# vwxyzjn/cleanrl

Measured on NVIDIA H100. Metric: env steps/sec (SPS) PPO Breakout num_envs=1024, higher is better.
Workload: dtype bf16

## Files before the change

### cleanrl_b200/csrc/tc_common.cuh

```cuda
#pragma once
#include <cuda_bf16.h>
#include <cstdint>
#include "tc_wgmma.cuh"

namespace b200rl { namespace tc {

__device__ __forceinline__ uint32_t smem_u32(const void* p) {
    return static_cast<uint32_t>(__cvta_generic_to_shared(p));
}

__device__ __forceinline__ void mbar_init(uint64_t* bar, uint32_t count) {
    asm volatile("mbarrier.init.shared::cta.b64 [%0], %1;" ::"r"(smem_u32(bar)), "r"(count) : "memory");
}
__device__ __forceinline__ void fence_barrier_init() {
    asm volatile("fence.mbarrier_init.release.cluster;" ::: "memory");
}
__device__ __forceinline__ bool mbar_try_wait(uint64_t* bar, uint32_t parity) {
    uint32_t ok;
    asm volatile(
        "{\n\t.reg .pred p;\n\t"
        "mbarrier.try_wait.parity.shared::cta.b64 p, [%1], %2;\n\t"
        "selp.u32 %0, 1, 0, p;\n\t}\n"
        : "=r"(ok)
        : "r"(smem_u32(bar)), "r"(parity)
        : "memory");
    return ok != 0;
}
#ifndef B200RL_WAIT_MODE
#define B200RL_WAIT_MODE 0
#endif
__device__ __forceinline__ bool mbar_try_wait_hint(uint64_t* bar, uint32_t parity, uint32_t ns) {
    uint32_t ok;
    asm volatile(
        "{\n\t.reg .pred p;\n\t"
        "mbarrier.try_wait.parity.shared::cta.b64 p, [%1], %2, %3;\n\t"
        "selp.u32 %0, 1, 0, p;\n\t}\n"
        : "=r"(ok)
        : "r"(smem_u32(bar)), "r"(parity), "r"(ns)
        : "memory");
    return ok != 0;
}
__device__ __forceinline__ void mbar_wait(uint64_t* bar, uint32_t parity) {
    if (mbar_try_wait(bar, parity)) return;
    const long long t0 = clock64();
#if B200RL_WAIT_MODE == 1
    while (!mbar_try_wait_hint(bar, parity, 1000000u)) {
#elif B200RL_WAIT_MODE == 2
    while (!mbar_try_wait(bar, parity)) {
        __nanosleep(40);
#else
    while (!mbar_try_wait(bar, parity)) {
#endif
        if (clock64() - t0 > (1ll << 33)) __trap();
    }
}

__device__ __forceinline__ void mbar_wait2(uint64_t* bar_a, uint32_t parity_a, uint64_t* bar_b, uint32_t parity_b) {
    const bool a = mbar_try_wait(bar_a, parity_a), b = mbar_try_wait(bar_b, parity_b);
    if (a && b) return;
    if (!a) mbar_wait(bar_a, parity_a);
    if (!b) mbar_wait(bar_b, parity_b);
}

__device__ __forceinline__ void st_global_32b(void* p, const int4& a, const int4& b) {
    reinterpret_cast<int4*>(p)[0] = a;
    reinterpret_cast<int4*>(p)[1] = b;
}

__device__ __forceinline__ void fence_proxy_async_smem() {
    asm volatile("fence.proxy.async.shared::cta;" ::: "memory");
}

constexpr uint64_t kDescSwizzle128 = 1ull << 62;
constexpr uint64_t kDescSwizzle64 = 2ull << 62;

__device__ __forceinline__ uint64_t desc_kmajor(uint32_t smem_addr) {
    return (uint64_t)((smem_addr & 0x3FFFFu) >> 4) | (1ull << 16) | (64ull << 32) | kDescSwizzle128;
}
__device__ __forceinline__ uint64_t desc_mnmajor(uint32_t smem_addr, uint32_t lbo_bytes) {
    return (uint64_t)((smem_addr & 0x3FFFFu) >> 4) | ((uint64_t)((lbo_bytes >> 4) & 0x3FFF) << 16) | (64ull << 32) |
           kDescSwizzle128;
}

template <int R>
__device__ __forceinline__ void stage_acc(float* st, int ld, int wg_tid, const float (&d)[R]) {
    const int row = ((wg_tid >> 5) << 4) + ((wg_tid & 31) >> 2), col = (wg_tid & 3) * 2;
#pragma unroll
    for (int j = 0; j < R / 4; ++j) {
        *reinterpret_cast<float2*>(st + row * ld + 8 * j + col) = make_float2(d[4 * j], d[4 * j + 1]);
        *reinterpret_cast<float2*>(st + (row + 8) * ld + 8 * j + col) = make_float2(d[4 * j + 2], d[4 * j + 3]);
    }
}
__device__ __forceinline__ void named_bar(int id, int n) { asm volatile("bar.sync %0, %1;" ::"r"(id), "r"(n) : "memory"); }

__device__ __forceinline__ uint32_t img_off(int r, int c) { return (uint32_t)(r * 128 + ((c ^ (r & 7)) << 4)); }

__device__ __forceinline__ uint32_t pack_bf16x2_relu(float lo, float hi) {
    uint32_t d;
    asm("cvt.rn.relu.bf16x2.f32 %0, %1, %2;" : "=r"(d) : "f"(hi), "f"(lo));
    return d;
}
__device__ __forceinline__ uint32_t pack_bf16x2(float lo, float hi) {
    __nv_bfloat162 v = __floats2bfloat162_rn(lo, hi);
    return *reinterpret_cast<uint32_t*>(&v);
}

}}

namespace b200rl { namespace tc {
__device__ __forceinline__ void cp_async16(uint32_t smem_addr, const void* gptr, uint32_t src_bytes) {
    asm volatile("cp.async.cg.shared.global [%0], [%1], 16, %2;" ::"r"(smem_addr), "l"(gptr), "r"(src_bytes) : "memory");
}
__device__ __forceinline__ void cp_async_commit() { asm volatile("cp.async.commit_group;" ::: "memory"); }
template <int N>
__device__ __forceinline__ void cp_async_wait() { asm volatile("cp.async.wait_group %0;" ::"n"(N) : "memory"); }
__device__ __forceinline__ void mbar_arrive(uint64_t* bar) {
    asm volatile("mbarrier.arrive.shared::cta.b64 _, [%0];" ::"r"(smem_u32(bar)) : "memory");
}
}}

namespace b200rl { namespace tc {
__device__ __forceinline__ void tma_load_2d(uint32_t smem_dst, const void* tmap, int x, int y, uint64_t* bar) {
    asm volatile("cp.async.bulk.tensor.2d.shared::cluster.global.mbarrier::complete_tx::bytes [%0], [%1, {%2, %3}], [%4];"
                 ::"r"(smem_dst), "l"(reinterpret_cast<uint64_t>(tmap)), "r"(x), "r"(y), "r"(smem_u32(bar))
                 : "memory");
}
__device__ __forceinline__ void tma_load_3d(uint32_t smem_dst, const void* tmap, int x, int y, int z, uint64_t* bar) {
    asm volatile("cp.async.bulk.tensor.3d.shared::cluster.global.mbarrier::complete_tx::bytes [%0], [%1, {%2, %3, %4}], [%5];"
                 ::"r"(smem_dst), "l"(reinterpret_cast<uint64_t>(tmap)), "r"(x), "r"(y), "r"(z), "r"(smem_u32(bar))
                 : "memory");
}
__device__ __forceinline__ void mbar_arrive_expect_tx(uint64_t* bar, uint32_t bytes) {
    asm volatile("mbarrier.arrive.expect_tx.shared::cta.b64 _, [%0], %1;" ::"r"(smem_u32(bar)), "r"(bytes) : "memory");
}
__device__ __forceinline__ void tma_prefetch_desc(const void* tmap) {
    asm volatile("prefetch.tensormap [%0];" ::"l"(reinterpret_cast<uint64_t>(tmap)) : "memory");
}
}}
```

### cleanrl_b200/csrc/tc_conv1_u8.cuh

```cuda
#pragma once
#include "tc_base.cuh"
#include <cuda_fp16.h>
#include "tc_conv_win.cuh"

namespace b200rl {
using namespace tc;

__device__ __forceinline__ uint64_t desc_kmajor_sw64(uint32_t smem_addr) {
    return (uint64_t)((smem_addr & 0x3FFFFu) >> 4) | (1ull << 16) | (32ull << 32) | kDescSwizzle64;
}
__device__ __forceinline__ uint64_t desc_mnmajor_sw64(uint32_t smem_addr, uint32_t lbo) {
    return (uint64_t)((smem_addr & 0x3FFFFu) >> 4) | ((uint64_t)((lbo >> 4) & 0x3FFF) << 16) | (32ull << 32) | kDescSwizzle64;
}
__device__ __forceinline__ uint32_t img64_off(int r, int c) { return (uint32_t)(r * 64 + ((c ^ ((r >> 1) & 3)) << 4)); }
__global__ void __launch_bounds__(256) tc_frames_to_s2d_u8(const uint8_t* __restrict__ obs, const int64_t* __restrict__ rows, int64_t n,
                                                           uint8_t* __restrict__ out_rm, uint8_t* __restrict__ out_cm) {
    __shared__ __align__(16) uint8_t plane[7056];
    const int64_t i = blockIdx.x >> 2;
    const int c = blockIdx.x & 3;
    const int64_t img = rows ? rows[i] : i;
    const int4* src = reinterpret_cast<const int4*>(obs + img * 28224 + c * 7056);
    for (int t = threadIdx.x; t < 441; t += 256) reinterpret_cast<int4*>(plane)[t] = __ldg(src + t);
    __syncthreads();
    for (int pos = threadIdx.x; pos < 441; pos += 256) {
// ... 77 lines not shown
    if (tid == 0) {
        for (int s = 0; s < STAGES; ++s) { mbar_init(&full_bar[s], 1); mbar_init(&empty_bar[s], 8); }
        fence_barrier_init();
        tma_prefetch_desc(&tmA);
    }
    for (int idx = tid; idx < NTAPS * BN * 4; idx += blockDim.x) {
        const int c16 = idx & 3;
        const int t = (idx >> 2) & 3;
        const int r = idx >> 4;
        *reinterpret_cast<int4*>(sW + t * B_CHUNK + img64_off(r, c16)) = ldg16(p.limbs + r * 256 + t * 64 + c16 * 16);
    }
    if (tid < 32) { s_sc[tid] = p.sc[32 + tid]; s_bias[tid] = p.bias[tid]; }
    fence_proxy_async_smem();
    __syncthreads();
    const int tile_begin = (int)(((int64_t)total_tiles * blockIdx.x) / gridDim.x);
    const int tile_end = (int)(((int64_t)total_tiles * (blockIdx.x + 1)) / gridDim.x);

    if (warp == 0) {
        if (tid == 0) {
            uint32_t q = 0;
            int z_next = 0;
            if (tile_begin < tile_end) {
                const int img = tile_begin >> 1;
                z_next = p.rows ? (int)__ldg(p.rows + img) : img;
            }
            for (int tile = tile_begin; tile < tile_end; ++tile, ++q) {
                const uint32_t s = q % STAGES;
                const int z = z_next;
                if (tile + 1 < tile_end) {
                    const int img = (tile + 1) >> 1;
                    z_next = p.rows ? (int)__ldg(p.rows + img) : img;
                }
                if (q >= (uint32_t)STAGES) mbar_wait(&empty_bar[s], ((q / STAGES) - 1) & 1);
                mbar_arrive_expect_tx(&full_bar[s], (uint32_t)STAGE_BYTES);
                tma_load_3d(smem_u32(sRing + (size_t)s * STAGE_BYTES), &tmA, 0, (tile & 1) * 128, z, &full_bar[s]);
            }
        }
    } else if (warp >= 4) {
        const int wg = (warp - 4) >> 2, wt = tid & 127, lane = tid & 31, qd = lane & 3;
        const uint32_t w_base = smem_u32(sW);
        constexpr int off[4] = {0, 1, 21, 22};
        int acc[2][32];
#pragma unroll
        for (int e = 0; e < 2; ++e)
#pragma unroll
            for (int c = 0; c < 32; ++c) acc[e][c] = 0;
        for (int tile = tile_begin; tile < tile_end; ++tile) {
            const uint32_t q = (uint32_t)(tile - tile_begin), s = q % STAGES;
            mbar_wait(&full_bar[s], (q / STAGES) & 1);
            wgmma_fence();
            const uint32_t win = smem_u32(sRing + (size_t)s * STAGE_BYTES) + (uint32_t)(wg * 64 * 128);
#pragma unroll
            for (int e = 0; e < 2; ++e) {
#pragma unroll
                for (int t = 0; t < NTAPS; ++t) {
                    const int po = e + off[t];
                    const uint64_t a = desc_kmajor(win + (uint32_t)((po >> 1) * 128 + (po & 1) * 64));
                    const uint64_t b = desc_kmajor_sw64(w_base + (uint32_t)(t * B_CHUNK));
#pragma unroll
                    for (int kk = 0; kk < 2; ++kk) wgmma_u8s8_n64(acc[e], a + 2 * kk, b + 2 * kk, (t | kk) != 0 ? 1u : 0u);
                }
            }
            wgmma_commit();
            wgmma_wait<0>();
            wgmma_fence_operands(acc[0]);
            wgmma_fence_operands(acc[1]);
            if (lane == 0) mbar_arrive(&empty_bar[s]);
            const int i = tile >> 1;
#pragma unroll
            for (int e = 0; e < 2; ++e) {
#pragma unroll
                for (int hr = 0; hr < 2; ++hr) {
                    const int lrow = wg * 64 + ((wt >> 5) << 4) + (lane >> 2) + 8 * hr;
                    const int rem = 2 * (((tile & 1) << 7) + lrow) + e;
                    const int Y = (rem * 3121) >> 16, X = rem - Y * 21;
                    const bool valid = rem < 441 && Y < 20 && X < 20;
                    const int64_t cell = ((int64_t)i * 10 + (Y >> 1)) * 10 + (X >> 1);
                    const int cls = (Y & 1) * 2 + (X & 1);
                    uint32_t bits = 0u, pk[4];
#pragma unroll
                    for (int j = 0; j < 4; ++j) {
                        const int co = 8 * j + 2 * qd;
                        const float f0 = fmaf((float)(acc[e][4 * j + 2 * hr] * 128 + acc[e][4 * (j + 4) + 2 * hr]), s_sc[co], s_bias[co]);
                        const float f1 = fmaf((float)(acc[e][4 * j + 2 * hr + 1] * 128 + acc[e][4 * (j + 4) + 2 * hr + 1]), s_sc[co + 1],
                                              s_bias[co + 1]);
                        bits |= (f0 > 0.f ? 1u : 0u) << co;
                        bits |= (f1 > 0.f ? 1u : 0u) << (co + 1);
                        pk[j] = pack_bf16x2_relu(f0, f1);
                    }
                    bits |= __shfl_xor_sync(0xffffffffu, bits, 1);
                    bits |= __shfl_xor_sync(0xffffffffu, bits, 2);
                    if (valid) {
                        if (qd == 0) p.mask_out[cell * 4 + cls] = bits;
                        uint32_t* dst = reinterpret_cast<uint32_t*>(reinterpret_cast<uint8_t*>(p.out) + (cell * 4 + cls) * 64);
#pragma unroll
                        for (int j = 0; j < 4; ++j) dst[4 * j + qd] = pk[j];
                    }
                }
            }
        }
    }
}

struct Conv21BwdU8Params {
    const int64_t* rows;
    int n;
    int64_t rows_per_cta;
    const bf16* w2dg;
    const uint32_t* m1;
    float* ws;
    float* wsb;
};
constexpr int kC1WXStages = 6, kC21WinStages = 2;
constexpr int kC1WBlock = 64 * 128, kC1WYBytes = 128 * 64, kC1WYPadRows = 24, kC1WYPad = kC1WYPadRows * 64;
constexpr int kC1WShift = 21;
constexpr int kC21WinRows = 140, kC21WinBytes = 18 * 1024;
constexpr int kC21W2Bytes = 4 * 128 * 128;
constexpr int kC21ImgBytes = kC1WYPad + 4 * kC1WYBytes;
constexpr float kDact1Scale = 4096.0f;

__device__ __forceinline__ uint32_t prmt(uint32_t a, uint32_t b, uint32_t sel) {
    uint32_t d;
    asm("prmt.b32 %0, %1, %2, %3;" : "=r"(d) : "r"(a), "r"(b), "r"(sel));
    return d;
}
constexpr float kU8Bias = 1024.0f;


__device__ __forceinline__ uint32_t pair_f16_biased(const uint32_t (&w)[5], int j, bool up, uint32_t sel) {
    const uint32_t lo = up ? w[j + 1] : w[j];
    const uint32_t hi = up ? w[j + 2] : w[j + 1];
    return prmt(prmt(lo, hi, sel), 0x64646464u, 0x5140u);
}
__device__ __forceinline__ uint4 lds128(uint32_t addr) {
    uint4 v;
    asm volatile("ld.shared.v4.u32 {%0, %1, %2, %3}, [%4];" : "=r"(v.x), "=r"(v.y), "=r"(v.z), "=r"(v.w) : "r"(addr) : "memory");
    return v;
}
__device__ __forceinline__ uint32_t pack_f16x2_sat(float lo, float hi) {
    uint32_t d;
    asm("cvt.rn.satfinite.f16x2.f32 %0, %1, %2;" : "=r"(d) : "f"(hi), "f"(lo));
    return d;
}

__device__ __forceinline__ void sts32(uint32_t addr, uint32_t v) { asm volatile("st.shared.u32 [%0], %1;" ::"r"(addr), "r"(v) : "memory"); }
__device__ __forceinline__ void tma_store_3d(const void* tmap, uint32_t smem_src, int x, int y, int z) {
    asm volatile("cp.async.bulk.tensor.3d.global.shared::cta.bulk_group [%0, {%1, %2, %3}], [%4];"
                 ::"l"(reinterpret_cast<uint64_t>(tmap)), "r"(x), "r"(y), "r"(z), "r"(smem_src) : "memory");
}
__device__ __forceinline__ void bulk_commit() { asm volatile("cp.async.bulk.commit_group;" ::: "memory"); }
template <int N> __device__ __forceinline__ void bulk_wait_read() { asm volatile("cp.async.bulk.wait_group.read %0;" ::"n"(N) : "memory"); }
template <int N> __device__ __forceinline__ void bulk_wait() { asm volatile("cp.async.bulk.wait_group %0;" ::"n"(N) : "memory"); }

template <int R> __device__ __forceinline__ void setmaxnreg_dec() { asm volatile("setmaxnreg.dec.sync.aligned.u32 %0;" ::"n"(R)); }
template <int R> __device__ __forceinline__ void setmaxnreg_inc() { asm volatile("setmaxnreg.inc.sync.aligned.u32 %0;" ::"n"(R)); }
constexpr int kC1WRegsProducer = 40, kC21RegsDgrad = 128, kC1WRegsMma = 168;
static_assert(128 * kC1WRegsProducer + 128 * kC21RegsDgrad + 256 * kC1WRegsMma <= 65536, "register budgets exceed the SM");

constexpr int kC1WThreads = 512;
__global__ void __launch_bounds__(kC1WThreads, 1) tc_conv21_bwd_u8(const __grid_constant__ CUtensorMap tmX, const __grid_constant__ CUtensorMap tmWin,
                                                                 const __grid_constant__ CUtensorMap tmY, const Conv21BwdU8Params p) {
    constexpr int XS = kC1WXStages, WS = kC21WinStages;
    extern __shared__ uint8_t smem_raw[];
    __shared__ uint64_t xfull[XS], xempty[XS], wfull[WS], wempty[WS], yfull[2], yempty[2];
    __shared__ float sRed[32 * 32], sBias[32];
    uint8_t* smem = reinterpret_cast<uint8_t*>((reinterpret_cast<uintptr_t>(smem_raw) + 1023) & ~uintptr_t(1023));
    uint8_t* sW2 = smem;
    uint8_t* sWin = sW2 + kC21W2Bytes;
    uint8_t* sX = sWin + (size_t)WS * kC21WinBytes;
    uint8_t* sImg = sX + (size_t)XS * kC1WBlock;
    const int tid = threadIdx.x, warp = tid >> 5, lane = tid & 31;
    if (tid == 0) {
        for (int s = 0; s < XS; ++s) { mbar_init(&xfull[s], 1); mbar_init(&xempty[s], 12); }
        for (int s = 0; s < WS; ++s) { mbar_init(&wfull[s], 1); mbar_init(&wempty[s], 4); }
        for (int s = 0; s < 2; ++s) { mbar_init(&yfull[s], 1); mbar_init(&yempty[s], 8); }
        fence_barrier_init();
        tma_prefetch_desc(&tmX);
        tma_prefetch_desc(&tmWin);
        tma_prefetch_desc(&tmY);
    }
    for (int idx = tid; idx < 4 * 128 * 8; idx += blockDim.x) {
        const int c16 = idx & 7, r = (idx >> 3) & 127, t = idx >> 10;
        *reinterpret_cast<int4*>(sW2 + t * (128 * 128) + img_off(r, c16)) = ldg16(p.w2dg + r * 256 + t * 64 + c16 * 8);
    }
    for (int idx = tid; idx < 2 * kC21ImgBytes / 16; idx += blockDim.x) reinterpret_cast<int4*>(sImg)[idx] = make_int4(0, 0, 0, 0);
    fence_proxy_async_smem();
    __syncthreads();
    const int64_t M = (int64_t)p.n * 512;
    const int64_t m_begin = (int64_t)blockIdx.x * p.rows_per_cta;
    int64_t m_end = m_begin + p.rows_per_cta;
    if (m_end > M) m_end = M;
    const int nsteps = m_end > m_begin ? (int)((m_end - m_begin) >> 7) : 0;
    const int nimg = nsteps >> 2;
    const int64_t g0 = m_begin >> 7;
    const int img0 = (int)(m_begin >> 9);

    if (warp < 4) {
        setmaxnreg_dec<kC1WRegsProducer>();
        if (warp == 0 && lane == 0 && nsteps > 0) {
            auto image_of = [&](int64_t g) -> int {
                int64_t img = g >> 2;
                if (img >= p.n) img = p.n - 1;
                return p.rows ? (int)__ldg(p.rows + img) : (int)img;
            };
            int z = image_of(g0), z_next = image_of(g0 + 4);
            for (int k = 0; k <= nsteps; ++k) {
                const int64_t g = g0 + k;
                if (k > 0 && (g & 3) == 0) { z = z_next; z_next = image_of(g + 4); }
                const int xs = k % XS;
                if (k >= XS) mbar_wait(&xempty[xs], ((k / XS) - 1) & 1);
                mbar_arrive_expect_tx(&xfull[xs], (uint32_t)kC1WBlock);
                tma_load_3d(smem_u32(sX + (size_t)xs * kC1WBlock), &tmX, (int)(g & 3) * 128, 0, z, &xfull[xs]);
            }
        } else if (warp == 1 && lane == 0) {
            for (int j = 0; j < nimg; ++j) {
                const int s = j % WS;
                if (j >= WS) mbar_wait(&wempty[s], ((j / WS) - 1) & 1);
                mbar_arrive_expect_tx(&wfull[s], (uint32_t)(kC21WinRows * 128));
                tma_load_2d(smem_u32(sWin + (size_t)s * kC21WinBytes), &tmWin, 0, (img0 + j) * 121, &wfull[s]);
            }
        }
    } else if (warp < 8) {
        const int wt = tid - 128, lane4 = lane >> 2, qd = lane & 3;
        const uint32_t w_base = smem_u32(sW2);
        const int rq = wt >> 2, c16 = wt & 3;
        float bsum[8];
#pragma unroll
        for (int e = 0; e < 8; ++e) bsum[e] = 0.f;
        for (int j = 0; j < nimg; ++j) {
            const int i = img0 + j, buf = j & 1, s = j % WS;
            const uint32_t img = smem_u32(sImg + (size_t)buf * kC21ImgBytes) + kC1WYPad;
            mbar_wait(&wfull[s], (j / WS) & 1);
            if (j >= 2) mbar_wait(&yempty[buf], ((j >> 1) - 1) & 1);
            if (wt == 0) bulk_wait_read<1>();
            named_bar(1, 128);
#pragma unroll 1
            for (int h2 = 0; h2 < 2; ++h2) {
                float d[64];
                wgmma_fence();
                const uint32_t win = smem_u32(sWin + (size_t)s * kC21WinBytes) + (uint32_t)(h2 * 64 * 128);
                constexpr int shift[4] = {12, 11, 1, 0};
#pragma unroll
                for (int t = 0; t < 4; ++t) {
                    const uint64_t a = desc_kmajor(win + (uint32_t)shift[t] * 128u);
                    const uint64_t b = desc_kmajor(w_base + (uint32_t)(t * 128 * 128));
#pragma unroll
                    for (int kk = 0; kk < 4; ++kk) WgmmaBf16<128, 0, 0>::mma(d, a + 2 * kk, b + 2 * kk, (t | kk) != 0 ? 1u : 0u);
                }
                wgmma_commit();
                int pos[2];
                uint4 mb[2];
#pragma unroll
                for (int hr = 0; hr < 2; ++hr) {
                    const int r = h2 * 64 + ((wt >> 5) << 4) + lane4 + 8 * hr;
                    const int Y = (r * 5958) >> 16, X = r - Y * 11;
                    const bool valid = Y < 10 && X < 10;
                    pos[hr] = valid ? 2 * Y * 21 + 2 * X : -1;
                    mb[hr] = make_uint4(0u, 0u, 0u, 0u);
                    if (valid) {
                        const int4 t = ldg16(p.m1 + ((int64_t)i * 100 + Y * 10 + X) * 4);
                        mb[hr] = make_uint4((uint32_t)t.x, (uint32_t)t.y, (uint32_t)t.z, (uint32_t)t.w);
                    }
                }
                wgmma_wait<0>();
                wgmma_fence_operands(d);
                if (h2 == 1 && lane == 0) mbar_arrive(&wempty[s]);
#pragma unroll
                for (int hr = 0; hr < 2; ++hr) {
                    if (pos[hr] < 0) continue;
                    const uint32_t mw[4] = {mb[hr].x, mb[hr].y, mb[hr].z, mb[hr].w};
#pragma unroll
                    for (int jj = 0; jj < 16; ++jj) {
                        const int g = jj >> 2, c = 8 * (jj & 3) + 2 * qd;
                        float f0 = d[4 * jj + 2 * hr] * kDact1Scale, f1 = d[4 * jj + 2 * hr + 1] * kDact1Scale;
                        if (!((mw[g] >> c) & 1u)) f0 = 0.f;
                        if (!((mw[g] >> (c + 1)) & 1u)) f1 = 0.f;
                        const int q = pos[hr] + (g >> 1) * 21 + (g & 1);
                        sts32(img + img64_off(q, c >> 3) + (uint32_t)((c & 7) * 2), pack_f16x2_sat(f0, f1));
                    }
                }
            }
            fence_proxy_async_smem();
            named_bar(1, 128);
            if (wt == 0) {
                mbar_arrive(&yfull[buf]);
#pragma unroll
                for (int k = 0; k < 4; ++k) tma_store_3d(&tmY, img + (uint32_t)(k * kC1WYBytes), 0, k * 128, i);
                bulk_commit();
            }
#pragma unroll 1
            for (int st = 0; st < 4; ++st) {
#pragma unroll
                for (int ps = 0; ps < 4; ++ps) {
                    const uint4 v = lds128(img + (uint32_t)(st * kC1WYBytes) + img64_off(ps * 32 + rq, c16));
                    const uint32_t w[4] = {v.x, v.y, v.z, v.w};
#pragma unroll
                    for (int e = 0; e < 4; ++e) {
                        const float2 f = __half22float2(*reinterpret_cast<const __half2*>(&w[e]));
                        bsum[2 * e] += f.x;
                        bsum[2 * e + 1] += f.y;
                    }
                }
            }
        }
        if (wt == 0) bulk_wait<0>();
#pragma unroll
        for (int e = 0; e < 8; ++e) sRed[rq * 32 + c16 * 8 + e] = bsum[e];
        named_bar(1, 128);
// ... 107 lines not shown
```

### cleanrl_b200/csrc/tc_conv_win.cuh

```cuda
#pragma once
#include "tc_base.cuh"

namespace b200rl {
using namespace tc;

enum { WOUT_DENSE = 0, WOUT_S2D2 = 1, WOUT_DACT2 = 2, WOUT_DACT1 = 3 };
struct WinParams {
    const bf16* A;
    const int64_t* rows;
    int64_t M;
    int n, G, Wp;
    int tpi_shift;
    int64_t n_images;
    int ntaps;
    int shift[16];
    int WR;
    const bf16* Bw;
    int N;
    int vH, vW;
    int out_mode;
    bf16* out;
    bf16* out2;
    const uint32_t* mask_bits;
    uint32_t* mask_out;
// ... 97 lines not shown
#pragma unroll
            for (int t = 0; t < NTAPS; ++t) {
#pragma unroll
                for (int c = 0; c < CPR; ++c) {
                    const uint64_t a = desc_kmajor(win + (uint32_t)(c * IMG) + (uint32_t)p.shift[t] * 128u);
                    const uint64_t b = desc_kmajor(w_base + (uint32_t)((t * CPR + c) * B_CHUNK));
#pragma unroll
                    for (int kk = 0; kk < 4; ++kk)
                        WgmmaBf16<BN, 0, 0>::mma(d, a + 2 * kk, b + 2 * kk, (t | c | kk) != 0 ? 1u : 0u);
                }
            }
            wgmma_commit();
            const int Y = (int)(((uint32_t)rem * mW) >> 16), X = rem - Y * p.Wp;
            const bool valid = inside && (Y < p.vH) && (X < p.vW);
            int64_t o1 = 0, ob = 0;
            if (p.out_mode == WOUT_S2D2) {
                const int64_t cell = ((int64_t)i * 10 + (Y >> 1)) * 10 + (X >> 1);
                const int cls = (Y & 1) * 2 + (X & 1);
                o1 = cell * 128 + cls * 32; ob = cell * 4 + cls;
            } else {
                ob = ((int64_t)i * 100 + Y * 10 + X) * 4;
            }
            uint32_t mb[NW];
#pragma unroll
            for (int g = 0; g < NW; ++g) mb[g] = 0xFFFFFFFFu;
            if (p.mask_bits != nullptr && valid) {
                if (NW == 4) {
                    const int4 t = ldg16(p.mask_bits + ob);
                    mb[0] = (uint32_t)t.x; mb[1 % NW] = (uint32_t)t.y; mb[2 % NW] = (uint32_t)t.z; mb[3 % NW] = (uint32_t)t.w;
                } else if (NW == 2) {
                    const uint2 t = __ldg(reinterpret_cast<const uint2*>(p.mask_bits + ob));
                    mb[0] = t.x; mb[1 % NW] = t.y;
                } else {
                    mb[0] = __ldg(p.mask_bits + ob);
                }
            }
            wgmma_wait<0>();
            wgmma_fence_operands(d);
            if ((tid & 31) == 0) mbar_arrive(&empty_bar[s]);
            named_bar(1 + wg, 128);
            stage_acc(st, LDA, wt, d);
            named_bar(1 + wg, 128);
#pragma unroll
            for (int g = 0; g < NW; ++g) {
                if ((g & 1) != half) continue;
                if (!valid || g * 32 >= p.N) continue;
                uint32_t v[32];
#pragma unroll
                for (int e = 0; e < 8; ++e) {
                    const float4 f = *reinterpret_cast<const float4*>(st + lr * LDA + g * 32 + 4 * e);
                    v[4 * e] = __float_as_uint(f.x); v[4 * e + 1] = __float_as_uint(f.y);
                    v[4 * e + 2] = __float_as_uint(f.z); v[4 * e + 3] = __float_as_uint(f.w);
                }
                if (p.bias) {
                    const float4* bp = reinterpret_cast<const float4*>(p.bias + g * 32);
#pragma unroll
                    for (int e = 0; e < 8; ++e) {
                        const float4 bv = __ldg(bp + e);
                        v[4 * e] = __float_as_uint(fmaf(__uint_as_float(v[4 * e]), p.scale, bv.x));
                        v[4 * e + 1] = __float_as_uint(fmaf(__uint_as_float(v[4 * e + 1]), p.scale, bv.y));
                        v[4 * e + 2] = __float_as_uint(fmaf(__uint_as_float(v[4 * e + 2]), p.scale, bv.z));
                        v[4 * e + 3] = __float_as_uint(fmaf(__uint_as_float(v[4 * e + 3]), p.scale, bv.w));
                    }
                } else {
#pragma unroll
                    for (int e = 0; e < 32; ++e) v[e] = __float_as_uint(__uint_as_float(v[e]) * p.scale);
                }
                if (p.relu) {
                    uint32_t bits = 0u;
#pragma unroll
                    for (int e = 0; e < 32; ++e) {
                        const float f = __uint_as_float(v[e]);
                        bits |= (f > 0.f ? 1u : 0u) << e;
                    }
                    if (p.mask_out) p.mask_out[ob + g] = bits;
                }
                if (p.mask_bits) {
#pragma unroll
                    for (int e = 0; e < 32; ++e) if (!((mb[g] >> e) & 1u)) v[e] = 0u;
                }
                int4 w[4];
                if (p.relu) {
#pragma unroll
                    for (int e = 0; e < 4; ++e) {
                        w[e].x = (int)pack_bf16x2_relu(__uint_as_float(v[8 * e]), __uint_as_float(v[8 * e + 1]));
                        w[e].y = (int)pack_bf16x2_relu(__uint_as_float(v[8 * e + 2]), __uint_as_float(v[8 * e + 3]));
                        w[e].z = (int)pack_bf16x2_relu(__uint_as_float(v[8 * e + 4]), __uint_as_float(v[8 * e + 5]));
                        w[e].w = (int)pack_bf16x2_relu(__uint_as_float(v[8 * e + 6]), __uint_as_float(v[8 * e + 7]));
                    }
                } else {
#pragma unroll
                for (int e = 0; e < 4; ++e) {
                    w[e].x = (int)pack_bf16x2(__uint_as_float(v[8 * e]), __uint_as_float(v[8 * e + 1]));
                    w[e].y = (int)pack_bf16x2(__uint_as_float(v[8 * e + 2]), __uint_as_float(v[8 * e + 3]));
                    w[e].z = (int)pack_bf16x2(__uint_as_float(v[8 * e + 4]), __uint_as_float(v[8 * e + 5]));
                    w[e].w = (int)pack_bf16x2(__uint_as_float(v[8 * e + 6]), __uint_as_float(v[8 * e + 7]));
                }
                }
                if (p.out_mode == WOUT_DACT1) {
                    int4* brow = reinterpret_cast<int4*>(st + lr * LDA) + 8 * g + 4 * (g & 1);
#pragma unroll
                    for (int e = 0; e < 4; ++e) brow[e] = w[e];
                } else {
                    bf16* dst = p.out + o1 + g * 32;
                    st_global_32b(dst, w[0], w[1]);
                    st_global_32b(dst + 16, w[2], w[3]);
                }
            }
            if (p.out_mode == WOUT_DACT1) {
                if (half == 0)
                    *reinterpret_cast<int64_t*>(st + lr * LDA + BN) = valid ? ((int64_t)i * 441 + 2 * Y * 21 + 2 * X) * 32 : -1;
                named_bar(1 + wg, 128);
#pragma unroll
                for (int m = 0; m < 8; ++m) {
                    const int k = m * 128 + wt, g = (k >> 2) & 3, e = k & 3;
                    const float* srow = st + (k >> 4) * LDA;
                    const int64_t o = *reinterpret_cast<const int64_t*>(srow + BN);
                    if (o < 0) continue;
                    const int4 val = reinterpret_cast<const int4*>(srow)[8 * g + 4 * (g & 1) + e];
                    *reinterpret_cast<int4*>(p.out + o + (g >> 1) * 21 * 32 + (g & 1) * 32 + e * 8) = val;
                }
            }
        }
    }
}

template <int BN, int CPR, int STAGES, int NTAPS>
static int launch_conv_win(const WinParams& p, cudaStream_t s, const char* what) {
    if (p.ntaps != NTAPS) return fail(B200RL_ERR_INVALID_ARGUMENT, "%s: %d taps, kernel instance has %d", what, p.ntaps, NTAPS);
    if (p.out_mode != WOUT_S2D2 && p.out_mode != WOUT_DACT1)
        return fail(B200RL_ERR_INVALID_ARGUMENT, "%s: dense and conv3 data-gradient outputs run on tc_conv_win_t", what);
    if (p.out_mode == WOUT_DACT1 && (BN != 128 || p.N != 128))
        return fail(B200RL_ERR_INVALID_ARGUMENT, "%s: the conv2 data gradient stores 4 groups of 32 channels per cell", what);
    const size_t smem = (size_t)p.ntaps * CPR * BN * 128 + (size_t)STAGES * p.WR * 128 * CPR + conv_win_acc_bytes<BN>() + 1024;
    static SmemAttrCache attr;
    if (int rc = attr.ensure(tc_conv_win<BN, CPR, STAGES, NTAPS>, smem, what)) return rc;
    if ((int64_t)p.G * p.Wp >= 65536 || p.G < 1 || p.N % 32 != 0)
        return fail(B200RL_ERR_INVALID_ARGUMENT, "%s: grid %d x width %d outside the epilogue's multiply-shift range, or N %% 32 != 0", what, p.G, p.Wp);
    if (p.rows && !p.tpi_shift) return fail(B200RL_ERR_INVALID_ARGUMENT, "%s: the image gather needs image-aligned tiling", what);
    if (p.tpi_shift && (128 << p.tpi_shift) < p.G) return fail(B200RL_ERR_INVALID_ARGUMENT, "%s: tiles per image too small", what);
    const int total = p.tpi_shift ? (int)((int64_t)p.n << p.tpi_shift) : (int)ceil_div(p.M, 128);
    int grid = num_sms();
    if (grid > total) grid = total;
    CUtensorMap tmA;
    memset(&tmA, 0, sizeof(tmA));
    int rc;
    if (p.tpi_shift) rc = make_tmap_3d(&tmA, p.A, p.n_images, p.G, (int64_t)CPR * 64, p.WR, what);
    else rc = make_tmap_2d(&tmA, p.A, p.M, (int64_t)CPR * 64, p.WR, what);
    if (rc) return rc;
    tc_conv_win<BN, CPR, STAGES, NTAPS><<<grid, kConvWinThreads, smem, s>>>(tmA, p, total);
    return check_launch(what);
}

constexpr int kConvWinTThreads = 384;
constexpr int kConvWinTLds = 64 + 4;
template <int BP>
__host__ __device__ constexpr size_t conv_win_t_stage_bytes() { return (size_t)2 * BP * kConvWinTLds * sizeof(float); }

template <int R>
__device__ __forceinline__ void stage_acc_transposed(float* st, int wg_tid, const float (&d)[R]) {
    const int co = ((wg_tid >> 5) << 4) + ((wg_tid & 31) >> 2), pos = (wg_tid & 3) * 2;
#pragma unroll
    for (int j = 0; j < R / 4; ++j) {
        float* p0 = st + (8 * j + pos) * kConvWinTLds + co;
        p0[0] = d[4 * j];
        p0[kConvWinTLds] = d[4 * j + 1];
        p0[8] = d[4 * j + 2];
        p0[kConvWinTLds + 8] = d[4 * j + 3];
    }
}

template <int BP, int CPR, int STAGES, int NTAPS>
__global__ void __launch_bounds__(kConvWinTThreads, 1) tc_conv_win_t(const __grid_constant__ CUtensorMap tmA, const WinParams p,
                                                                     int total_tiles) {
    static_assert(BP % 128 == 0, "one thread per position row of a 128-row slice");
    static_assert(STAGES % 2 == 0, "each consumer warpgroup owns every other stage");
    constexpr int RPT = BP / 128;
    constexpr int A_CHUNK = 64 * 128;
    constexpr int LDS = kConvWinTLds;
    extern __shared__ uint8_t smem_raw[];
    __shared__ uint64_t full_bar[STAGES], empty_bar[STAGES];
    uint8_t* smem = reinterpret_cast<uint8_t*>((reinterpret_cast<uintptr_t>(smem_raw) + 1023) & ~uintptr_t(1023));
    const int tid = threadIdx.x, warp = tid >> 5;
    const int nchunks = NTAPS * CPR;
    const int K = nchunks * 64;
    const int IMG = p.WR * 128;
    const int STAGE_BYTES = IMG * CPR;
    uint8_t* sW = smem;
    uint8_t* sRing = smem + (size_t)nchunks * A_CHUNK;
    float* sAcc = reinterpret_cast<float*>(sRing + (size_t)STAGES * STAGE_BYTES);

    if (tid == 0) {
        for (int s = 0; s < STAGES; ++s) { mbar_init(&full_bar[s], 1); mbar_init(&empty_bar[s], 4); }
        fence_barrier_init();
        tma_prefetch_desc(&tmA);
    }
    for (int idx = tid; idx < nchunks * 64 * 8; idx += blockDim.x) {
        const int c16 = idx & 7;
        const int t = idx >> 3;
        const int r = t & 63, j = t >> 6;
        int4 v = make_int4(0, 0, 0, 0);
        if (r < p.N) v = ldg16(p.Bw + (int64_t)r * K + j * 64 + c16 * 8);
        *reinterpret_cast<int4*>(sW + (size_t)j * A_CHUNK + img_off(r, c16)) = v;
    }
    fence_proxy_async_smem();
    __syncthreads();
    const int tile_begin = (int)(((int64_t)total_tiles * blockIdx.x) / gridDim.x);
    const int tile_end = (int)(((int64_t)total_tiles * (blockIdx.x + 1)) / gridDim.x);

    if (warp == 0) {
        if (tid == 0) {
            uint32_t q = 0;
            for (int tile = tile_begin; tile < tile_end; ++tile, ++q) {
                const uint32_t s = q % STAGES;
                if (q >= (uint32_t)STAGES) mbar_wait(&empty_bar[s], ((q / STAGES) - 1) & 1);
                const uint32_t dst = smem_u32(sRing + (size_t)s * STAGE_BYTES);
                mbar_arrive_expect_tx(&full_bar[s], (uint32_t)STAGE_BYTES);
#pragma unroll
                for (int c = 0; c < CPR; ++c) tma_load_2d(dst + c * IMG, &tmA, c * 64, tile * BP, &full_bar[s]);
            }
        }
    } else if (warp >= 4) {
        const int wg = (warp - 4) >> 2, wt = tid & 127;
        float* st = sAcc + wg * BP * LDS;
        const uint32_t w_base = smem_u32(sW);
        const uint32_t mW = (65536u + (uint32_t)p.Wp - 1u) / (uint32_t)p.Wp;
        constexpr int NW = 2;
        float d[BP / 2];
#pragma unroll
        for (int e = 0; e < BP / 2; ++e) d[e] = 0.f;
        for (int tile = tile_begin + wg; tile < tile_end; tile += 2) {
            const uint32_t q = (uint32_t)(tile - tile_begin), s = q % STAGES;
            mbar_wait(&full_bar[s], (q / STAGES) & 1);
            wgmma_fence();
            const uint32_t win = smem_u32(sRing + (size_t)s * STAGE_BYTES);
#pragma unroll
            for (int t = 0; t < NTAPS; ++t) {
#pragma unroll
                for (int c = 0; c < CPR; ++c) {
                    const uint64_t b = desc_kmajor(win + (uint32_t)(c * IMG) + (uint32_t)p.shift[t] * 128u);
                    const uint64_t a = desc_kmajor(w_base + (uint32_t)((t * CPR + c) * A_CHUNK));
#pragma unroll
                    for (int kk = 0; kk < 4; ++kk)
                        WgmmaBf16<BP, 0, 0>::mma(d, a + 2 * kk, b + 2 * kk, (t | c | kk) != 0 ? 1u : 0u);
                }
            }
            wgmma_commit();
            bool valid[RPT];
            int64_t o1[RPT], o2[RPT], ob[RPT];
            uint32_t mb[RPT][NW];
#pragma unroll
            for (int rr = 0; rr < RPT; ++rr) {
                const int64_t r = (int64_t)tile * BP + rr * 128 + wt;
                const int i = (int)(r / p.G);
                const int rem = (int)(r - (int64_t)i * p.G);
                const int Y = (int)(((uint32_t)rem * mW) >> 16), X = rem - Y * p.Wp;
                valid[rr] = r < p.M && (Y < p.vH) && (X < p.vW);
                o2[rr] = 0;
                if (p.out_mode == WOUT_DENSE) {
                    const int64_t orow = ((int64_t)i * p.vH + Y) * p.vW + X;
                    o1[rr] = orow * p.N; ob[rr] = orow * (p.N >> 5);
                } else {
                    o1[rr] = ((int64_t)i * 100 + Y * 10 + X) * 64;
                    o2[rr] = ((int64_t)i * 121 + (Y + 1) * 11 + (X + 1)) * 64;
                    ob[rr] = ((int64_t)i * 81 + Y * 9 + X) * 2;
                }
                mb[rr][0] = mb[rr][1] = 0xFFFFFFFFu;
                if (p.mask_bits != nullptr && valid[rr]) {
                    const uint2 t = __ldg(reinterpret_cast<const uint2*>(p.mask_bits + ob[rr]));
                    mb[rr][0] = t.x; mb[rr][1] = t.y;
                }
            }
            wgmma_wait<0>();
            wgmma_fence_operands(d);
            if ((tid & 31) == 0) mbar_arrive(&empty_bar[s]);
            named_bar(1 + wg, 128);
            stage_acc_transposed(st, wt, d);
            named_bar(1 + wg, 128);
#pragma unroll
            for (int rr = 0; rr < RPT; ++rr) {
                float* srow = st + (rr * 128 + wt) * LDS;
#pragma unroll
                for (int g = 0; g < NW; ++g) {
                    if (!valid[rr] || g * 32 >= p.N) continue;
                    uint32_t v[32];
#pragma unroll
                    for (int e = 0; e < 8; ++e) {
                        const float4 f = *reinterpret_cast<const float4*>(srow + g * 32 + 4 * e);
                        v[4 * e] = __float_as_uint(f.x); v[4 * e + 1] = __float_as_uint(f.y);
                        v[4 * e + 2] = __float_as_uint(f.z); v[4 * e + 3] = __float_as_uint(f.w);
                    }
                    if (p.bias) {
                        const float4* bp = reinterpret_cast<const float4*>(p.bias + g * 32);
#pragma unroll
                        for (int e = 0; e < 8; ++e) {
                            const float4 bv = __ldg(bp + e);
                            v[4 * e] = __float_as_uint(fmaf(__uint_as_float(v[4 * e]), p.scale, bv.x));
                            v[4 * e + 1] = __float_as_uint(fmaf(__uint_as_float(v[4 * e + 1]), p.scale, bv.y));
                            v[4 * e + 2] = __float_as_uint(fmaf(__uint_as_float(v[4 * e + 2]), p.scale, bv.z));
                            v[4 * e + 3] = __float_as_uint(fmaf(__uint_as_float(v[4 * e + 3]), p.scale, bv.w));
                        }
                    } else {
#pragma unroll
                        for (int e = 0; e < 32; ++e) v[e] = __float_as_uint(__uint_as_float(v[e]) * p.scale);
                    }
                    if (p.relu) {
                        uint32_t bits = 0u;
#pragma unroll
                        for (int e = 0; e < 32; ++e) bits |= (__uint_as_float(v[e]) > 0.f ? 1u : 0u) << e;
                        if (p.mask_out) p.mask_out[ob[rr] + g] = bits;
                    }
                    if (p.mask_bits) {
#pragma unroll
                        for (int e = 0; e < 32; ++e) if (!((mb[rr][g] >> e) & 1u)) v[e] = 0u;
                    }
                    int4 w[4];
                    if (p.relu) {
#pragma unroll
                        for (int e = 0; e < 4; ++e) {
                            w[e].x = (int)pack_bf16x2_relu(__uint_as_float(v[8 * e]), __uint_as_float(v[8 * e + 1]));
                            w[e].y = (int)pack_bf16x2_relu(__uint_as_float(v[8 * e + 2]), __uint_as_float(v[8 * e + 3]));
                            w[e].z = (int)pack_bf16x2_relu(__uint_as_float(v[8 * e + 4]), __uint_as_float(v[8 * e + 5]));
                            w[e].w = (int)pack_bf16x2_relu(__uint_as_float(v[8 * e + 6]), __uint_as_float(v[8 * e + 7]));
                        }
                    } else {
#pragma unroll
                        for (int e = 0; e < 4; ++e) {
                            w[e].x = (int)pack_bf16x2(__uint_as_float(v[8 * e]), __uint_as_float(v[8 * e + 1]));
                            w[e].y = (int)pack_bf16x2(__uint_as_float(v[8 * e + 2]), __uint_as_float(v[8 * e + 3]));
                            w[e].z = (int)pack_bf16x2(__uint_as_float(v[8 * e + 4]), __uint_as_float(v[8 * e + 5]));
                            w[e].w = (int)pack_bf16x2(__uint_as_float(v[8 * e + 6]), __uint_as_float(v[8 * e + 7]));
                        }
                    }
                    int4* brow = reinterpret_cast<int4*>(srow) + 4 * g;
#pragma unroll
                    for (int e = 0; e < 4; ++e) brow[e] = w[e];
                }
                *reinterpret_cast<longlong2*>(srow + 64) = make_longlong2(valid[rr] ? o1[rr] : -1, o2[rr]);
            }
            named_bar(1 + wg, 128);
#pragma unroll
            for (int m = 0; m < BP / 16; ++m) {
                const int k = m * 128 + wt, part = k & 7;
                const float* srow = st + (k >> 3) * LDS;
                const longlong2 off = *reinterpret_cast<const longlong2*>(srow + 64);
                if (off.x < 0) continue;
                const int4 val = reinterpret_cast<const int4*>(srow)[part];
                *reinterpret_cast<int4*>(p.out + off.x + part * 8) = val;
                if (p.out_mode == WOUT_DACT2) *reinterpret_cast<int4*>(p.out2 + off.y + part * 8) = val;
            }
        }
    }
}

template <int BP, int CPR, int STAGES, int NTAPS>
static int launch_conv_win_t(WinParams p, cudaStream_t s, const char* what) {
    if (p.ntaps != NTAPS) return fail(B200RL_ERR_INVALID_ARGUMENT, "%s: %d taps, kernel instance has %d", what, p.ntaps, NTAPS);
    if (p.N != 64) return fail(B200RL_ERR_INVALID_ARGUMENT, "%s: N = %d, the kernel computes 64 output channels", what, p.N);
    if ((int64_t)p.G * p.Wp >= 65536 || p.G < 1)
        return fail(B200RL_ERR_INVALID_ARGUMENT, "%s: grid %d x width %d outside the epilogue's multiply-shift range", what, p.G, p.Wp);
    if (p.rows || p.tpi_shift) return fail(B200RL_ERR_INVALID_ARGUMENT, "%s: the channel-major kernel walks a contiguous linear grid", what);
    if (p.out_mode != WOUT_DENSE && p.out_mode != WOUT_DACT2)
        return fail(B200RL_ERR_INVALID_ARGUMENT, "%s: only bf16 dense and conv3 data-gradient outputs in this kernel", what);
    int maxs = 0;
    for (int t = 0; t < NTAPS; ++t) maxs = p.shift[t] > maxs ? p.shift[t] : maxs;
    p.WR = (BP + maxs + 7) & ~7;
    if (p.WR > 256) return fail(B200RL_ERR_INVALID_ARGUMENT, "%s: window of %d rows exceeds a TMA box", what, p.WR);
    const size_t smem = (size_t)NTAPS * CPR * 64 * 128 + (size_t)STAGES * p.WR * 128 * CPR + conv_win_t_stage_bytes<BP>() + 1024;
    static SmemAttrCache attr;
    if (int rc = attr.ensure(tc_conv_win_t<BP, CPR, STAGES, NTAPS>, smem, what)) return rc;
    const int total = (int)ceil_div(p.M, BP);
    int grid = num_sms();
    if (grid > total) grid = total;
    CUtensorMap tmA;
    memset(&tmA, 0, sizeof(tmA));
    if (int rc = make_tmap_2d(&tmA, p.A, p.M, (int64_t)CPR * 64, p.WR, what)) return rc;
    tc_conv_win_t<BP, CPR, STAGES, NTAPS><<<grid, kConvWinTThreads, smem, s>>>(tmA, p, total);
    return check_launch(what);
}

}
```

Before: 1.192 million.

## Split conv window kernel into producer, MMA and dedicated epilogue warpgroups

Restructures the channel-major windowed conv kernel into five warpgroups: a TMA producer, two MMA warpgroups and two epilogue warpgroups. They hand off through staged and freed mbarriers on double-buffered accumulator staging, so the next tile's MMA can overlap the current tile's epilogue. Registers are rebalanced with setmaxnreg, and weights are loaded by TMA instead of a cooperative global-to-shared copy. Bias is cached in shared memory, and BP is restricted to 128 with a 32-bit position index. The cost is more threads and tighter per-thread register budgets, which risks spills, and a more complex barrier protocol.

```diff
diff --git a/cleanrl_b200/csrc/tc_common.cuh b/cleanrl_b200/csrc/tc_common.cuh
--- a/cleanrl_b200/csrc/tc_common.cuh
+++ b/cleanrl_b200/csrc/tc_common.cuh
@@ -93,6 +93,9 @@
 }
 __device__ __forceinline__ void named_bar(int id, int n) { asm volatile("bar.sync %0, %1;" ::"r"(id), "r"(n) : "memory"); }
 
+template <int R> __device__ __forceinline__ void setmaxnreg_dec() { asm volatile("setmaxnreg.dec.sync.aligned.u32 %0;" ::"n"(R)); }
+template <int R> __device__ __forceinline__ void setmaxnreg_inc() { asm volatile("setmaxnreg.inc.sync.aligned.u32 %0;" ::"n"(R)); }
+
 __device__ __forceinline__ uint32_t img_off(int r, int c) { return (uint32_t)(r * 128 + ((c ^ (r & 7)) << 4)); }
 
 __device__ __forceinline__ uint32_t pack_bf16x2_relu(float lo, float hi) {
diff --git a/cleanrl_b200/csrc/tc_conv1_u8.cuh b/cleanrl_b200/csrc/tc_conv1_u8.cuh
--- a/cleanrl_b200/csrc/tc_conv1_u8.cuh
+++ b/cleanrl_b200/csrc/tc_conv1_u8.cuh
@@ -253,8 +253,6 @@
 template <int N> __device__ __forceinline__ void bulk_wait_read() { asm volatile("cp.async.bulk.wait_group.read %0;" ::"n"(N) : "memory"); }
 template <int N> __device__ __forceinline__ void bulk_wait() { asm volatile("cp.async.bulk.wait_group %0;" ::"n"(N) : "memory"); }
 
-template <int R> __device__ __forceinline__ void setmaxnreg_dec() { asm volatile("setmaxnreg.dec.sync.aligned.u32 %0;" ::"n"(R)); }
-template <int R> __device__ __forceinline__ void setmaxnreg_inc() { asm volatile("setmaxnreg.inc.sync.aligned.u32 %0;" ::"n"(R)); }
 constexpr int kC1WRegsProducer = 40, kC21RegsDgrad = 128, kC1WRegsMma = 168;
 static_assert(128 * kC1WRegsProducer + 128 * kC21RegsDgrad + 256 * kC1WRegsMma <= 65536, "register budgets exceed the SM");
 
diff --git a/cleanrl_b200/csrc/tc_conv_win.cuh b/cleanrl_b200/csrc/tc_conv_win.cuh
--- a/cleanrl_b200/csrc/tc_conv_win.cuh
+++ b/cleanrl_b200/csrc/tc_conv_win.cuh
@@ -273,10 +273,15 @@
     return check_launch(what);
 }
 
-constexpr int kConvWinTThreads = 384;
 constexpr int kConvWinTLds = 64 + 4;
 template <int BP>
 __host__ __device__ constexpr size_t conv_win_t_stage_bytes() { return (size_t)2 * BP * kConvWinTLds * sizeof(float); }
+
+constexpr int kConvWinTThreads = 640;
+constexpr int kConvWinTRegsLaunch = (65536 / kConvWinTThreads) & ~7;
+constexpr int kConvWinTRegsProducer = 24, kConvWinTRegsMma = 112, kConvWinTRegsEpi = 112;
+static_assert(128 * kConvWinTRegsProducer + 256 * kConvWinTRegsMma + 256 * kConvWinTRegsEpi <= kConvWinTRegsLaunch * kConvWinTThreads,
+              "register budgets exceed what the CTA launches with");
 
 template <int R>
 __device__ __forceinline__ void stage_acc_transposed(float* st, int wg_tid, const float (&d)[R]) {
@@ -292,19 +297,20 @@
 }
 
 template <int BP, int CPR, int STAGES, int NTAPS>
-__global__ void __launch_bounds__(kConvWinTThreads, 1) tc_conv_win_t(const __grid_constant__ CUtensorMap tmA, const WinParams p,
-                                                                     int total_tiles) {
-    static_assert(BP % 128 == 0, "one thread per position row of a 128-row slice");
-    static_assert(STAGES % 2 == 0, "each consumer warpgroup owns every other stage");
-    constexpr int RPT = BP / 128;
+__global__ void __launch_bounds__(kConvWinTThreads, 1)
+    tc_conv_win_t(const __grid_constant__ CUtensorMap tmA, const __grid_constant__ CUtensorMap tmW, const WinParams p,
+                  int total_tiles) {
+    static_assert(BP == 128, "one epilogue thread per position row");
+    static_assert(STAGES % 2 == 0, "each MMA warpgroup owns every other stage");
     constexpr int A_CHUNK = 64 * 128;
     constexpr int LDS = kConvWinTLds;
+    constexpr int NW = 2;
     extern __shared__ uint8_t smem_raw[];
-    __shared__ uint64_t full_bar[STAGES], empty_bar[STAGES];
+    __shared__ uint64_t full_bar[STAGES], empty_bar[STAGES], staged_bar[2], freed_bar[2], w_bar;
+    __shared__ __align__(16) float s_bias[2][64];
     uint8_t* smem = reinterpret_cast<uint8_t*>((reinterpret_cast<uintptr_t>(smem_raw) + 1023) & ~uintptr_t(1023));
-    const int tid = threadIdx.x, warp = tid >> 5;
+    const int tid = threadIdx.x, warp = tid >> 5, wgi = warp >> 2, wt = tid & 127;
     const int nchunks = NTAPS * CPR;
-    const int K = nchunks * 64;
     const int IMG = p.WR * 128;
     const int STAGE_BYTES = IMG * CPR;
     uint8_t* sW = smem;
@@ -313,24 +319,21 @@
 
     if (tid == 0) {
         for (int s = 0; s < STAGES; ++s) { mbar_init(&full_bar[s], 1); mbar_init(&empty_bar[s], 4); }
+        for (int b = 0; b < 2; ++b) { mbar_init(&staged_bar[b], 128); mbar_init(&freed_bar[b], 128); }
+        mbar_init(&w_bar, 1);
         fence_barrier_init();
         tma_prefetch_desc(&tmA);
+        tma_prefetch_desc(&tmW);
     }
-    for (int idx = tid; idx < nchunks * 64 * 8; idx += blockDim.x) {
-        const int c16 = idx & 7;
-        const int t = idx >> 3;
-        const int r = t & 63, j = t >> 6;
-        int4 v = make_int4(0, 0, 0, 0);
-        if (r < p.N) v = ldg16(p.Bw + (int64_t)r * K + j * 64 + c16 * 8);
-        *reinterpret_cast<int4*>(sW + (size_t)j * A_CHUNK + img_off(r, c16)) = v;
-    }
-    fence_proxy_async_smem();
     __syncthreads();
     const int tile_begin = (int)(((int64_t)total_tiles * blockIdx.x) / gridDim.x);
     const int tile_end = (int)(((int64_t)total_tiles * (blockIdx.x + 1)) / gridDim.x);
 
-    if (warp == 0) {
-        if (tid == 0) {
+    if (wgi == 0) {
+        setmaxnreg_dec<kConvWinTRegsProducer>();
+        if (tid == 0 && tile_begin < tile_end) {
+            mbar_arrive_expect_tx(&w_bar, (uint32_t)(nchunks * A_CHUNK));
+            for (int j = 0; j < nchunks; ++j) tma_load_2d(smem_u32(sW + (size_t)j * A_CHUNK), &tmW, j * 64, 0, &w_bar);
             uint32_t q = 0;
             for (int tile = tile_begin; tile < tile_end; ++tile, ++q) {
                 const uint32_t s = q % STAGES;
@@ -341,16 +344,17 @@
                 for (int c = 0; c < CPR; ++c) tma_load_2d(dst + c * IMG, &tmA, c * 64, tile * BP, &full_bar[s]);
             }
         }
-    } else if (warp >= 4) {
-        const int wg = (warp - 4) >> 2, wt = tid & 127;
+    } else if (wgi <= 2) {
+        setmaxnreg_inc<kConvWinTRegsMma>();
+        const int wg = wgi - 1;
         float* st = sAcc + wg * BP * LDS;
         const uint32_t w_base = smem_u32(sW);
-        const uint32_t mW = (65536u + (uint32_t)p.Wp - 1u) / (uint32_t)p.Wp;
-        constexpr int NW = 2;
         float d[BP / 2];
 #pragma unroll
         for (int e = 0; e < BP / 2; ++e) d[e] = 0.f;
-        for (int tile = tile_begin + wg; tile < tile_end; tile += 2) {
+        if (tile_begin + wg < tile_end) mbar_wait(&w_bar, 0);
+        uint32_t k = 0;
+        for (int tile = tile_begin + wg; tile < tile_end; tile += 2, ++k) {
             const uint32_t q = (uint32_t)(tile - tile_begin), s = q % STAGES;
             mbar_wait(&full_bar[s], (q / STAGES) & 1);
             wgmma_fence();
@@ -367,109 +371,113 @@
                 }
             }
             wgmma_commit();
-            bool valid[RPT];
-            int64_t o1[RPT], o2[RPT], ob[RPT];
-            uint32_t mb[RPT][NW];
-#pragma unroll
-            for (int rr = 0; rr < RPT; ++rr) {
-                const int64_t r = (int64_t)tile * BP + rr * 128 + wt;
-                const int i = (int)(r / p.G);
-                const int rem = (int)(r - (int64_t)i * p.G);
-                const int Y = (int)(((uint32_t)rem * mW) >> 16), X = rem - Y * p.Wp;
-                valid[rr] = r < p.M && (Y < p.vH) && (X < p.vW);
-                o2[rr] = 0;
-                if (p.out_mode == WOUT_DENSE) {
-                    const int64_t orow = ((int64_t)i * p.vH + Y) * p.vW + X;
-                    o1[rr] = orow * p.N; ob[rr] = orow * (p.N >> 5);
-                } else {
-                    o1[rr] = ((int64_t)i * 100 + Y * 10 + X) * 64;
-                    o2[rr] = ((int64_t)i * 121 + (Y + 1) * 11 + (X + 1)) * 64;
-                    ob[rr] = ((int64_t)i * 81 + Y * 9 + X) * 2;
-                }
-                mb[rr][0] = mb[rr][1] = 0xFFFFFFFFu;
-                if (p.mask_bits != nullptr && valid[rr]) {
-                    const uint2 t = __ldg(reinterpret_cast<const uint2*>(p.mask_bits + ob[rr]));
-                    mb[rr][0] = t.x; mb[rr][1] = t.y;
-                }
-            }
             wgmma_wait<0>();
             wgmma_fence_operands(d);
             if ((tid & 31) == 0) mbar_arrive(&empty_bar[s]);
-            named_bar(1 + wg, 128);
+            if (k > 0) mbar_wait(&freed_bar[wg], (k - 1) & 1);
             stage_acc_transposed(st, wt, d);
-            named_bar(1 + wg, 128);
-#pragma unroll
-            for (int rr = 0; rr < RPT; ++rr) {
-                float* srow = st + (rr * 128 + wt) * LDS;
-#pragma unroll
-                for (int g = 0; g < NW; ++g) {
-                    if (!valid[rr] || g * 32 >= p.N) continue;
-                    uint32_t v[32];
+            mbar_arrive(&staged_bar[wg]);
+        }
+    } else {
+        setmaxnreg_inc<kConvWinTRegsEpi>();
+        const int b = wgi - 3;
+        float* st = sAcc + b * BP * LDS;
+        float* srow = st + wt * LDS;
+        const uint32_t mW = (65536u + (uint32_t)p.Wp - 1u) / (uint32_t)p.Wp;
+        float* sb = s_bias[b];
+        if (p.bias && wt < 64) sb[wt] = __ldg(p.bias + wt);
+        named_bar(1 + b, 128);
+        uint32_t k = 0;
+        for (int tile = tile_begin + b; tile < tile_end; tile += 2, ++k) {
+            const uint32_t r = (uint32_t)tile * BP + (uint32_t)wt;
+            const int i = (int)(r / (uint32_t)p.G);
+            const int rem = (int)(r - (uint32_t)i * (uint32_t)p.G);
+            const int Y = (int)(((uint32_t)rem * mW) >> 16), X = rem - Y * p.Wp;
+            const bool valid = (int64_t)r < p.M && (Y < p.vH) && (X < p.vW);
+            int64_t o1, o2 = 0, ob;
+            if (p.out_mode == WOUT_DENSE) {
+                const int64_t orow = ((int64_t)i * p.vH + Y) * p.vW + X;
+                o1 = orow * p.N; ob = orow * (p.N >> 5);
+            } else {
+                o1 = ((int64_t)i * 100 + Y * 10 + X) * 64;
+                o2 = ((int64_t)i * 121 + (Y + 1) * 11 + (X + 1)) * 64;
+                ob = ((int64_t)i * 81 + Y * 9 + X) * 2;
+            }
+            uint32_t mb[NW] = {0xFFFFFFFFu, 0xFFFFFFFFu};
+            if (p.mask_bits != nullptr && valid) {
+                const uint2 t = __ldg(reinterpret_cast<const uint2*>(p.mask_bits + ob));
+                mb[0] = t.x; mb[1] = t.y;
+            }
+            mbar_wait(&staged_bar[b], k & 1);
+#pragma unroll
+            for (int g = 0; g < NW; ++g) {
+                if (!valid || g * 32 >= p.N) continue;
+                uint32_t v[32];
+#pragma unroll
+                for (int e = 0; e < 8; ++e) {
+                    const float4 f = *reinterpret_cast<const float4*>(srow + g * 32 + 4 * e);
+                    v[4 * e] = __float_as_uint(f.x); v[4 * e + 1] = __float_as_uint(f.y);
+                    v[4 * e + 2] = __float_as_uint(f.z); v[4 * e + 3] = __float_as_uint(f.w);
+                }
+                if (p.bias) {
+                    const float4* bp = reinterpret_cast<const float4*>(sb + g * 32);
 #pragma unroll
                     for (int e = 0; e < 8; ++e) {
-                        const float4 f = *reinterpret_cast<const float4*>(srow + g * 32 + 4 * e);
-                        v[4 * e] = __float_as_uint(f.x); v[4 * e + 1] = __float_as_uint(f.y);
-                        v[4 * e + 2] = __float_as_uint(f.z); v[4 * e + 3] = __float_as_uint(f.w);
+                        const float4 bv = bp[e];
+                        v[4 * e] = __float_as_uint(fmaf(__uint_as_float(v[4 * e]), p.scale, bv.x));
+                        v[4 * e + 1] = __float_as_uint(fmaf(__uint_as_float(v[4 * e + 1]), p.scale, bv.y));
+                        v[4 * e + 2] = __float_as_uint(fmaf(__uint_as_float(v[4 * e + 2]), p.scale, bv.z));
+                        v[4 * e + 3] = __float_as_uint(fmaf(__uint_as_float(v[4 * e + 3]), p.scale, bv.w));
                     }
-                    if (p.bias) {
-                        const float4* bp = reinterpret_cast<const float4*>(p.bias + g * 32);
-#pragma unroll
-                        for (int e = 0; e < 8; ++e) {
-                            const float4 bv = __ldg(bp + e);
-                            v[4 * e] = __float_as_uint(fmaf(__uint_as_float(v[4 * e]), p.scale, bv.x));
-                            v[4 * e + 1] = __float_as_uint(fmaf(__uint_as_float(v[4 * e + 1]), p.scale, bv.y));
-                            v[4 * e + 2] = __float_as_uint(fmaf(__uint_as_float(v[4 * e + 2]), p.scale, bv.z));
-                            v[4 * e + 3] = __float_as_uint(fmaf(__uint_as_float(v[4 * e + 3]), p.scale, bv.w));
-                        }
-                    } else {
-#pragma unroll
-                        for (int e = 0; e < 32; ++e) v[e] = __float_as_uint(__uint_as_float(v[e]) * p.scale);
+                } else {
+#pragma unroll
+                    for (int e = 0; e < 32; ++e) v[e] = __float_as_uint(__uint_as_float(v[e]) * p.scale);
+                }
+                if (p.relu) {
+                    uint32_t bits = 0u;
+#pragma unroll
+                    for (int e = 0; e < 32; ++e) bits |= (__uint_as_float(v[e]) > 0.f ? 1u : 0u) << e;
+                    if (p.mask_out) p.mask_out[ob + g] = bits;
+                }
+                if (p.mask_bits) {
+#pragma unroll
+                    for (int e = 0; e < 32; ++e) if (!((mb[g] >> e) & 1u)) v[e] = 0u;
+                }
+                int4 w[4];
+                if (p.relu) {
+#pragma unroll
+                    for (int e = 0; e < 4; ++e) {
+                        w[e].x = (int)pack_bf16x2_relu(__uint_as_float(v[8 * e]), __uint_as_float(v[8 * e + 1]));
+                        w[e].y = (int)pack_bf16x2_relu(__uint_as_float(v[8 * e + 2]), __uint_as_float(v[8 * e + 3]));
+                        w[e].z = (int)pack_bf16x2_relu(__uint_as_float(v[8 * e + 4]), __uint_as_float(v[8 * e + 5]));
+                        w[e].w = (int)pack_bf16x2_relu(__uint_as_float(v[8 * e + 6]), __uint_as_float(v[8 * e + 7]));
                     }
-                    if (p.relu) {
-                        uint32_t bits = 0u;
-#pragma unroll
-                        for (int e = 0; e < 32; ++e) bits |= (__uint_as_float(v[e]) > 0.f ? 1u : 0u) << e;
-                        if (p.mask_out) p.mask_out[ob[rr] + g] = bits;
+                } else {
+#pragma unroll
+                    for (int e = 0; e < 4; ++e) {
+                        w[e].x = (int)pack_bf16x2(__uint_as_float(v[8 * e]), __uint_as_float(v[8 * e + 1]));
+                        w[e].y = (int)pack_bf16x2(__uint_as_float(v[8 * e + 2]), __uint_as_float(v[8 * e + 3]));
+                        w[e].z = (int)pack_bf16x2(__uint_as_float(v[8 * e + 4]), __uint_as_float(v[8 * e + 5]));
+                        w[e].w = (int)pack_bf16x2(__uint_as_float(v[8 * e + 6]), __uint_as_float(v[8 * e + 7]));
                     }
-                    if (p.mask_bits) {
-#pragma unroll
-                        for (int e = 0; e < 32; ++e) if (!((mb[rr][g] >> e) & 1u)) v[e] = 0u;
-                    }
-                    int4 w[4];
-                    if (p.relu) {
-#pragma unroll
-                        for (int e = 0; e < 4; ++e) {
-                            w[e].x = (int)pack_bf16x2_relu(__uint_as_float(v[8 * e]), __uint_as_float(v[8 * e + 1]));
-                            w[e].y = (int)pack_bf16x2_relu(__uint_as_float(v[8 * e + 2]), __uint_as_float(v[8 * e + 3]));
-                            w[e].z = (int)pack_bf16x2_relu(__uint_as_float(v[8 * e + 4]), __uint_as_float(v[8 * e + 5]));
-                            w[e].w = (int)pack_bf16x2_relu(__uint_as_float(v[8 * e + 6]), __uint_as_float(v[8 * e + 7]));
-                        }
-                    } else {
-#pragma unroll
-                        for (int e = 0; e < 4; ++e) {
-                            w[e].x = (int)pack_bf16x2(__uint_as_float(v[8 * e]), __uint_as_float(v[8 * e + 1]));
-                            w[e].y = (int)pack_bf16x2(__uint_as_float(v[8 * e + 2]), __uint_as_float(v[8 * e + 3]));
-                            w[e].z = (int)pack_bf16x2(__uint_as_float(v[8 * e + 4]), __uint_as_float(v[8 * e + 5]));
-                            w[e].w = (int)pack_bf16x2(__uint_as_float(v[8 * e + 6]), __uint_as_float(v[8 * e + 7]));
-                        }
-                    }
-                    int4* brow = reinterpret_cast<int4*>(srow) + 4 * g;
-#pragma unroll
-                    for (int e = 0; e < 4; ++e) brow[e] = w[e];
-                }
-                *reinterpret_cast<longlong2*>(srow + 64) = make_longlong2(valid[rr] ? o1[rr] : -1, o2[rr]);
-            }
-            named_bar(1 + wg, 128);
+                }
+                int4* brow = reinterpret_cast<int4*>(srow) + 4 * g;
+#pragma unroll
+                for (int e = 0; e < 4; ++e) brow[e] = w[e];
+            }
+            *reinterpret_cast<longlong2*>(srow + 64) = make_longlong2(valid ? o1 : -1, o2);
+            named_bar(1 + b, 128);
 #pragma unroll
             for (int m = 0; m < BP / 16; ++m) {
-                const int k = m * 128 + wt, part = k & 7;
-                const float* srow = st + (k >> 3) * LDS;
-                const longlong2 off = *reinterpret_cast<const longlong2*>(srow + 64);
+                const int kq = m * 128 + wt, part = kq & 7;
+                const float* orow = st + (kq >> 3) * LDS;
+                const longlong2 off = *reinterpret_cast<const longlong2*>(orow + 64);
                 if (off.x < 0) continue;
-                const int4 val = reinterpret_cast<const int4*>(srow)[part];
+                const int4 val = reinterpret_cast<const int4*>(orow)[part];
                 *reinterpret_cast<int4*>(p.out + off.x + part * 8) = val;
                 if (p.out_mode == WOUT_DACT2) *reinterpret_cast<int4*>(p.out2 + off.y + part * 8) = val;
             }
+            mbar_arrive(&freed_bar[b]);
         }
     }
 }
@@ -480,6 +488,8 @@
     if (p.N != 64) return fail(B200RL_ERR_INVALID_ARGUMENT, "%s: N = %d, the kernel computes 64 output channels", what, p.N);
     if ((int64_t)p.G * p.Wp >= 65536 || p.G < 1)
         return fail(B200RL_ERR_INVALID_ARGUMENT, "%s: grid %d x width %d outside the epilogue's multiply-shift range", what, p.G, p.Wp);
+    if (p.M + BP >= (int64_t)1 << 31)
+        return fail(B200RL_ERR_INVALID_ARGUMENT, "%s: %lld grid positions exceed the epilogue's 32-bit position index", what, (long long)p.M);
     if (p.rows || p.tpi_shift) return fail(B200RL_ERR_INVALID_ARGUMENT, "%s: the channel-major kernel walks a contiguous linear grid", what);
     if (p.out_mode != WOUT_DENSE && p.out_mode != WOUT_DACT2)
         return fail(B200RL_ERR_INVALID_ARGUMENT, "%s: only bf16 dense and conv3 data-gradient outputs in this kernel", what);
@@ -493,10 +503,12 @@
     const int total = (int)ceil_div(p.M, BP);
     int grid = num_sms();
     if (grid > total) grid = total;
-    CUtensorMap tmA;
+    CUtensorMap tmA, tmW;
     memset(&tmA, 0, sizeof(tmA));
+    memset(&tmW, 0, sizeof(tmW));
     if (int rc = make_tmap_2d(&tmA, p.A, p.M, (int64_t)CPR * 64, p.WR, what)) return rc;
-    tc_conv_win_t<BP, CPR, STAGES, NTAPS><<<grid, kConvWinTThreads, smem, s>>>(tmA, p, total);
+    if (int rc = make_tmap_2d(&tmW, p.Bw, 64, (int64_t)NTAPS * CPR * 64, 64, what)) return rc;
+    tc_conv_win_t<BP, CPR, STAGES, NTAPS><<<grid, kConvWinTThreads, smem, s>>>(tmA, tmW, p, total);
     return check_launch(what);
 }
 
```

Measured after the change: 1.224 million (median of 6 runs). 2.7% higher.
